# xuqingkuang/FluidFramework

Hardware: AMD Instinct MI355X
Metric: sequenced merge-tree ops applied/sec (node) at 100K docs; % HBM roofline (higher is better)
Workload: dtype int32; 1 GPU; C3: 100000 docs/GPU x 32 clients x 1024 sequenced ops/doc (BASELINE.json configs[2]), full merge-tree apply incl. zamboni; docs_total=100000, docs_per_gpu=100000, docs_rank0=100000, ops_per_doc=1024, ops_per_launch=32, parallelism=hash-routed docs x1 (splitmix64(docId) mod 1; no collective in apply), comm=LocalComm

## Files before the change

fluidframework_amd/build.py:

```python
import os
import subprocess
import sys

HERE = os.path.dirname(os.path.abspath(__file__))
CSRC = os.path.join(HERE, 'csrc')
LIB = os.path.join(HERE, 'libmtgpu.so')
SOURCES = ['mt_apply.hip', 'mt_apply_reg.hip', 'mt_service.hip', 'mt_refs.hip', 'mt_intervals.hip', 'mt_text.hip', 'mt_markers.hip', 'mt_deli.hip', 'mt_engine.cpp',
           'mt_queries.cpp', 'mt_readout.cpp', 'mt_comm.cpp']
HEADERS = ['mt_state.h', 'mt_wave.h', 'mt_checksum.h', 'mt_synth.h', 'mt_seqwin.h', 'mt_view.h', 'mt_marker.h', 'mt_launch.h',
           'mt_engine_impl.h', 'mt_scratch.h', '../../include/mtgpu.h']
HIPCC = os.environ.get('HIPCC', '/opt/rocm/bin/hipcc')
ARCH = os.environ.get('PYTORCH_ROCM_ARCH', 'gfx950')


def needs_build():
    if not os.path.exists(LIB):
        return True
    t = os.path.getmtime(LIB)
    return any(os.path.getmtime(os.path.join(CSRC, f)) > t for f in SOURCES + HEADERS
               if os.path.exists(os.path.join(CSRC, f)))


def build(force=False, verbose=False, prof=False):
    lib = LIB.replace('libmtgpu.so', 'libmtgpu_prof.so') if prof else LIB
    if not prof and not force and not needs_build():
        return LIB
    from concurrent.futures import ThreadPoolExecutor
    objdir = os.path.join(HERE, 'build')
    os.makedirs(objdir, exist_ok=True)
    srcs = [f for f in SOURCES if os.path.exists(os.path.join(CSRC, f))]
    flags = [f'--offload-arch={ARCH}', '-O3', '-std=c++17', '-fPIC', '-Wall', '-Wno-unused-function',
             '-Wno-unused-result', '-Wno-unused-value'] + os.environ.get('MTGPU_EXTRA_FLAGS', '').split()

    stamp = ' '.join(flags + (['-DMT_PROF'] if prof else []))
    hdr_t = max(os.path.getmtime(os.path.join(CSRC, h)) for h in HEADERS if os.path.exists(os.path.join(CSRC, h)))

    def fresh(f, obj):
        try:
            t = os.path.getmtime(obj)
            with open(obj + '.flags') as fh:
                same = fh.read() == stamp
        except OSError:
            return False
        return same and t > os.path.getmtime(os.path.join(CSRC, f)) and t > hdr_t

    def cc(f):
        obj = os.path.join(objdir, f + ('.prof.o' if prof else '.o'))
        if not force and fresh(f, obj):
            return obj
        cmd = [HIPCC] + flags + (['-DMT_PROF'] if prof else []) + ['-c', os.path.join(CSRC, f), '-o', obj]
        if verbose:
            print(' '.join(cmd))
        subprocess.check_call(cmd)
        with open(obj + '.flags', 'w') as fh:
            fh.write(stamp)
        return obj

    with ThreadPoolExecutor(max_workers=len(srcs)) as ex:
        objs = list(ex.map(cc, srcs))
    subprocess.check_call([HIPCC, f'--offload-arch={ARCH}', '-shared', '-o', lib + '.tmp'] + objs +
                          ['-L/opt/rocm/lib', '-lrccl', '-Wl,-rpath,/opt/rocm/lib'])
    os.replace(lib + '.tmp', lib)
    return lib
# ... 28 lines not shown
```

fluidframework_amd/csrc/mt_apply_reg.hip:

```cpp
#include <hip/hip_runtime.h>
#include <stdint.h>

#include "../../include/mtgpu.h"
#include "mt_seqwin.h"
#include "mt_launch.h"
#include "mt_state.h"
#include "mt_wave.h"

namespace mtr {

constexpr int kMaxNodes = 8;
constexpr int kTextGranularity = 256;
constexpr int kNarrowClients = 32;
constexpr int kC64Clients = 63;
constexpr uint32_t kLenBits = 17;
constexpr uint32_t kLenMask = (1u << kLenBits) - 1;
constexpr uint32_t kNoId = 0x7FFFu;
constexpr uint32_t kEmptyLi = kNoId << kLenBits;
constexpr uint32_t F_RM = (uint32_t)MT_SF_REMOVED << 16;
constexpr uint32_t F_PDEF = (uint32_t)MT_SF_PDEF << 16;
constexpr uint32_t F_NL = (uint32_t)MT_SF_NL << 16;
constexpr uint32_t F_HASNL = (uint32_t)MT_SF_HASNL << 16;
constexpr uint32_t F_MARKER = (uint32_t)MT_SF_MARKER << 16;
constexpr uint32_t F_NLQ = 1u << 21;
constexpr uint32_t kEmptyCf = 0xFFu;
constexpr uint32_t kOrgShift = 22;
constexpr uint16_t kDead = 0xFFFFu;

#define MT_GLOB __attribute__((address_space(1)))
#define MT_KARG __attribute__((address_space(4)))
template <class T>
MT_DEV MT_GLOB T* gp(T* p) { return (MT_GLOB T*)p; }
typedef const MT_KARG mt_gstate KGState;
typedef uint32_t EvWords __attribute__((ext_vector_type(4)));
MT_DEV void put_event(MT_GLOB mt_event* p, int32_t seq, int op, unsigned flags, int leaf, int pos, uint32_t len,
                      uint32_t pmask = 0, uint32_t pv01 = 0, uint32_t pv23 = 0, uint32_t pv45 = 0, uint32_t pv67 = 0) {
    static_assert(sizeof(mt_event) == 96 && offsetof(mt_event, pvals) == 24, "mt_event");
    MT_GLOB EvWords* q = reinterpret_cast<MT_GLOB EvWords*>(p);
    const EvWords z = {0u, 0u, 0u, 0u};
    q[0] = EvWords{(uint32_t)seq, ((uint32_t)op & 0xFFu) | ((flags & 0xFFu) << 8), (uint32_t)leaf, (uint32_t)pos};
    q[1] = EvWords{len, pmask, pv01, pv23};
    q[2] = EvWords{pv45, pv67, 0u, 0u};
    q[3] = z;
    q[4] = z;
    q[5] = z;
}

MT_DEV int uni(int v) { return __builtin_amdgcn_readfirstlane(v); }
MT_DEV uint32_t uniu(uint32_t v) { return (uint32_t)__builtin_amdgcn_readfirstlane((int)v); }
MT_DEV int shr1(int v, int fill) { return __builtin_amdgcn_update_dpp(fill, v, 0x138, 0xf, 0xf, false); }
MT_DEV int shl1(int v, int fill) { return __builtin_amdgcn_update_dpp(fill, v, 0x130, 0xf, 0xf, false); }
MT_DEV int wave_total(int v) { return wave_last(wave_incl_scan(v)); }

enum { P_LOAD, P_SCAN, P_BOUND, P_INSERT, P_RANGE, P_ZAMBONI, P_SCOUR, P_STORE, P_OPS, P_ZPOP, P_REPACK,
       P_B_GET, P_B_BLK, P_B_TXT, P_B_INS, P_N_SCOUR, P_N_UNLINK, P_N_APPEND, P_N_SPLIT,
       P_COMPACT, P_N_COMPACT, P_N_APPBYTES, P_B_SRCH, P_B_LEAF, P_OP, P_NSLOT };
[[maybe_unused]] constexpr int kProfStride = 32;
#ifdef MT_PROF
__device__ unsigned long long mt_prof_acc[16 * kProfStride];
MT_DEV uint64_t prof_now() {
    unsigned long long t;
    __builtin_amdgcn_sched_barrier(0);
    asm volatile("s_memtime %0\n\ts_waitcnt lgkmcnt(0)" : "=s"(t)::"memory");
    __builtin_amdgcn_sched_barrier(0);
    return t;
}
#ifndef MT_PROF_ONLY
#define MT_PROF_ONLY -1
#endif
#define PROF_ON(s) (MT_PROF_ONLY < 0 || MT_PROF_ONLY == (s))
#define PROF_BEGIN(v, s) const uint64_t v = PROF_ON(s) ? prof_now() : 0
#define PROF_BEGIN2(v, s1, s2) const uint64_t v = (PROF_ON(s1) || PROF_ON(s2)) ? prof_now() : 0
#define PROF_END(arr, slot, v) \
    do {                       \
        if (PROF_ON(slot)) arr[slot] += prof_now() - (v); \
    } while (0)
#define PROF_CNT(slot, v) prof[slot] += (v)
#else
#define PROF_BEGIN(v, s)
#define PROF_BEGIN2(v, s1, s2)
#define PROF_END(arr, slot, v)
#define PROF_CNT(slot, v)
#endif

template <int K>
struct RLds {
    static constexpr int CAP = 64 * K;
    static constexpr int LB = CAP / 2 > 128 ? CAP / 2 : 128;
    static constexpr int IB = CAP / 8 + 8 > 40 ? CAP / 8 + 8 : 40;
    static constexpr int H = CAP / 2 + 64 > 192 ? CAP / 2 + 64 : 192;
    uint64_t props[CAP];
    union {
        int32_t scr[CAP + 1];
        uint32_t tln[CAP + 1];
    };
    int32_t hseq[H];
    uint16_t toff[CAP];
    uint16_t hslot[H];
    uint8_t ibcnt[MT_MAXLEV - 1][IB];
    uint8_t lbsc[LB + 1];
    int32_t nb[MT_MAXLEV];
    uint32_t zr[4 * kMaxNodes];
    uint64_t dum[64];
};

struct Elem {
    uint32_t sw;
    uint32_t rsq;
    uint32_t li, cf, ov, oh;
    int32_t cum;
};
struct Cut {
    uint32_t lli, lcf, rli;
    int32_t pos;
};

template <int K, bool W = false, bool EV = false>
struct RWave {
    using L = RLds<K>;
    static constexpr int CAP = L::CAP;
    static constexpr uint32_t kAll = (1u << K) - 1u;
    typedef int32_t VI __attribute__((ext_vector_type(K)));
    typedef uint32_t VU __attribute__((ext_vector_type(K)));
    typedef uint32_t U4 __attribute__((ext_vector_type(4)));
    typedef uint32_t U2 __attribute__((ext_vector_type(2)));
    L& s;
    const int lane;
    uint8_t* const abase;
    const uint32_t textcap;

    static constexpr bool PK = K > MT_SW_EXACT_K;
    VU sw;
    VU rsq;
    VU li, cf, ov;
    VU oh;
    VI cum;
    int ns, nlive, nb0, nlev, heap_n, cur_seq, min_seq, err, err_seq, next_id;
    int32_t base_seq;
    uint32_t text_top, text_half;
    bool dirty;
    uint32_t pb;
    uint32_t bsm, lvm, sc0, sc1;
    MT_GLOB mt_event* evp = nullptr;
    uint32_t evcap = 0;
    int evn = 0;
    int32_t evseq = 0;
#ifdef MT_PROF
    uint64_t prof[P_NSLOT] = {};
#endif

    MT_DEV RWave(L& lds, uint8_t* a, uint32_t tc)
        : s(lds), lane(lane_id()), abase(a), textcap(tc), dirty(false) {}
    MT_DEV uint8_t* arena() const { return abase + (size_t)text_half * textcap; }

    MT_DEV int idx(int j) const { return lane * K + j; }

    MT_DEV void fail(int code, int32_t sq) {
        if (err == 0) {
            err = code;
            err_seq = sq;
        }
    }
    MT_DEV static uint32_t len_of(uint32_t l) { return l & kLenMask; }
    MT_DEV static uint32_t id_of(uint32_t l) { return l >> kLenBits; }
    MT_DEV uint32_t lim_of(int32_t R) const { return PK ? mt_sw_lim(R, base_seq) : (uint32_t)R; }
    MT_DEV uint32_t key_of(int32_t S) const { return PK ? mt_sw_off(S, base_seq) : (uint32_t)S; }
    MT_DEV static bool key_le(uint32_t a, uint32_t lim) { return PK ? a <= lim : (int32_t)a <= (int32_t)lim; }
    MT_DEV bool seq_le(int j, uint32_t lim) const { return PK ? mt_sw_seq_le(sw[j], lim) != 0 : (int32_t)sw[j] <= (int32_t)lim; }
    MT_DEV bool rseq_le(int j, uint32_t lim) const { return PK ? mt_sw_rseq_le(sw[j], lim) != 0 : (int32_t)rsq[j] <= (int32_t)lim; }
    MT_DEV bool rseq_eq(int j, uint32_t key) const { return PK ? mt_sw_rseq_eq(sw[j], key) != 0 : rsq[j] == key; }

    MT_DEV uint32_t bs_bits() const { return bsm; }
    MT_DEV uint32_t live_bits() const { return lvm; }
    MT_DEV uint32_t kbit(int k) const {
        const int r = k - lane * K;
        return (r >= 0 && r < K) ? (1u << r) : 0u;
    }
    MT_DEV int sc_of(int a) const {
        const int r = uni(a % K);
        return __builtin_amdgcn_readlane((int)(((sc0 >> r) & 1u) | (((sc1 >> r) & 1u) << 1)), a / K);
    }
    MT_DEV void set_sc(int a, int v) {
        const uint32_t b = kbit(a);
        sc0 = (v & 1) ? (sc0 | b) : (sc0 & ~b);
        sc1 = (v & 2) ? (sc1 | b) : (sc1 & ~b);
    }
    MT_DEV void set_bs(int a, bool on) {
        const uint32_t b = kbit(a);
        bsm = on ? (bsm | b) : (bsm & ~b);
    }
    MT_DEV static uint32_t shift_mask(uint32_t m, uint32_t lo, bool at, bool above, int r, bool bit) {
        const uint32_t c = (uint32_t)shr1((int)((m >> (K - 1)) & 1u), 0);
        return (m & lo) | (((m & ~lo) << 1) & kAll) | ((at && bit) ? (1u << r) : 0u) | (above ? c : 0u);
    }
    MT_DEV void mask_shift(int p, bool bs, int scv, bool live) {
        const uint32_t lo = below(p);
        const int r = p - lane * K;
        const bool at = r >= 0 && r < K, above = r < 0;
        bsm = shift_mask(bsm, lo, at, above, r, bs);
        lvm = shift_mask(lvm, lo, at, above, r, live);
        sc0 = shift_mask(sc0, lo, at, above, r, (scv & 1) != 0);
        sc1 = shift_mask(sc1, lo, at, above, r, (scv & 2) != 0);
    }
    MT_DEV uint32_t below(int k) const {
        const int r = k - lane * K;
        return r <= 0 ? 0u : (r >= K ? kAll : ((1u << r) - 1u));
    }
    MT_DEV int nth_slot(uint32_t m, int r) const {
// ... 317 lines not shown

    MT_DEV bool insert_at(int k, int a, int en, const Elem& e, int32_t sq, const Cut& cut, bool dup) {
        if (ns + 1 > CAP) return fail(MT_DERR_CAPACITY, sq), false;
        const bool front = !dup && k == a;
        PROF_BEGIN(ti0, P_B_INS);
        const int scv = front ? sc_of(a) : 0;
        shift_in<true>(k, e, front, scv, true, dup);
        if (dup) patch_cut(k, cut);
        if (front) {
            set_bs(k + 1, false);
            set_sc(k + 1, MT_SC_UNDEF);
        }
        PROF_END(prof, P_B_INS, ti0);
        nlive += 1;
        PROF_BEGIN(ti1, P_B_LEAF);
        const bool over = live_in(a, en + 1) >= kMaxNodes;
        PROF_END(prof, P_B_LEAF, ti1);
        if (!over) return true;
        PROF_BEGIN(ti2, P_COMPACT);
        PROF_CNT(P_N_COMPACT, 1);
        const bool r = split_leaf(a, en + 1, sq);
        PROF_END(prof, P_COMPACT, ti2);
        return r;
    }
    MT_DEV int alloc_id(int32_t sq) {
        if (next_id >= CAP) {
            fail(MT_DERR_CAPACITY, sq);
            return -1;
        }
        return next_id++;
    }

    MT_DEV void arena_sync() {
        if (dirty) {
            __threadfence_block();
            dirty = false;
        }
    }
    MT_DEV void arena_copy(uint32_t dst, uint32_t src, uint32_t cnt) {
        arena_sync();
        for (uint32_t base = 0; base < cnt; base += 64) {
            const uint32_t i = base + lane;
            if (i < cnt) arena()[dst + i] = arena()[src + i];
        }
        dirty = true;
    }
    MT_DEV void compact_text(int nid) {
        PROF_BEGIN(tc, P_COMPACT);
        PROF_CNT(P_N_COMPACT, 1);
        arena_sync();
        const uint8_t* src0 = arena();
        uint8_t* dst = abase + (size_t)(text_half ^ 1u) * textcap;
        uint32_t carry = 0;
        for (int base = 0; base < nid; base += 64) {
            const int i = base + lane;
            const uint32_t l = i < nid ? s.tln[i] : 0u;
            const uint32_t incl = (uint32_t)wave_incl_scan((int)l);
            const uint32_t at = carry + incl - l;
            if (l) {
                const uint8_t* src = src0 + s.toff[i];
#pragma clang loop unroll(disable) vectorize(disable)
                for (uint32_t q = 0; q < l; q++) dst[at + q] = src[q];
                s.toff[i] = (uint16_t)at;
            }
            carry += (uint32_t)wave_last((int)incl);
        }
        dirty = true;
        wave_sync();
        text_half ^= 1u;
        text_top = carry;
        PROF_END(prof, P_COMPACT, tc);
    }
    MT_DEV bool arena_reserve(uint32_t need, int32_t sq, int nid) {
        if (text_top + need <= textcap) return true;
        compact_text(nid);
        if (text_top + need <= textcap) return true;
        fail(MT_DERR_TEXT_ARENA, sq);
        return false;
    }

    MT_DEV bool split_prep(int pos, int32_t sq, Cut& c, int& k1, int& ba, int& be) {
        PROF_BEGIN(ts0, P_B_SRCH);
        int cs = cs0();
        int hitj = -1;
#pragma unroll
        for (int j = 0; j < K; j++) {
            if (cs < pos && pos < cum[j]) hitj = j;
            cs = cum[j];
        }
        const uint64_t m = wave_ballot(hitj >= 0);
        PROF_END(prof, P_B_SRCH, ts0);
        if (!m) return false;
        PROF_CNT(P_N_SPLIT, 1);
        PROF_BEGIN(tb0, P_B_GET);
        const int lk = first_lane(m);
        const int jk = uni(__builtin_amdgcn_readlane(hitj, lk));
        const int k = lk * K + jk;
        const uint32_t eli = (uint32_t)__builtin_amdgcn_readlane((int)li[jk], lk);
        const uint32_t ecf = (uint32_t)__builtin_amdgcn_readlane((int)cf[jk], lk);
        const int32_t ecum = __builtin_amdgcn_readlane(cum[jk], lk);
        PROF_END(prof, P_B_GET, tb0);
        const uint32_t len = len_of(eli);
        const int off = pos - (ecum - (int)len);
        const int t = alloc_id(sq);
        if (t < 0) return false;
        PROF_BEGIN(tb1, P_B_BLK);
        ba = block_start(k);
        be = next_start(k);
        PROF_END(prof, P_B_BLK, tb1);
        PROF_BEGIN(tb2, P_B_TXT);
        const uint32_t id = id_of(eli);
        const uint64_t pid = s.props[id];
        const uint32_t to = uniu(s.toff[id]);
        if (lane == 0) {
            s.props[t] = pid;
            s.toff[t] = (uint16_t)(to + (uint32_t)off);
            s.tln[id] = (uint32_t)off;
            s.tln[t] = len - (uint32_t)off;
        }
        c.lli = (uint32_t)off | (id << kLenBits);
        c.lcf = (ecf & F_HASNL) ? ((ecf & ~F_NL) | F_NLQ) : (ecf & ~(F_NL | F_NLQ));
        c.rli = (len - (uint32_t)off) | ((uint32_t)t << kLenBits);
        c.pos = pos;
        wave_sync();
        PROF_END(prof, P_B_TXT, tb2);
        if constexpr (EV) {
            const int lf = live_before(k);
            emit(MT_EV_SPLIT, MT_EVF_FIRST, lf, -1, (uint32_t)off);
            emit(MT_EV_SPLIT, 0u, lf + 1, -1, len - (uint32_t)off);
        }
        k1 = k + 1;
        return true;
    }

    MT_DEV bool heap_push(int32_t key, int id, int32_t sq) {
        if (heap_n + 1 >= L::H) return fail(MT_DERR_CAPACITY, sq), false;
        const int k0 = heap_n + 1;
        const int anc = lane < 31 ? (k0 >> (lane + 1)) : 0;
        const bool has = anc >= 1;
        const int32_t av = has ? s.hseq[anc] : 0;
        const uint16_t as = has ? s.hslot[anc] : (uint16_t)0;
        const int up = first_lane(wave_ballot(!has || av - key <= 0));
        wave_sync();
        if (lane < up) {
            const int child = k0 >> lane;
            s.hseq[child] = av;
            s.hslot[child] = as;
        }
        if (lane == 0) {
            s.hseq[k0 >> up] = key;
            s.hslot[k0 >> up] = (uint16_t)id;
        }
        heap_n = heap_n + 1;
        wave_sync();
        return true;
    }
    MT_DEV int heap_pop() {
        const int cnt = heap_n - 1;
        int k = 1, id = 0;
        int32_t x = 0;
        uint32_t xs = 0;
        const int r = lane + 2;
        const int dep = 31 - __builtin_clz((uint32_t)r);
        for (bool first = true, more = true; more; first = false) {
            const int node = (k << dep) + (r - (1 << dep));
            const bool ok = lane < 62 && node <= cnt;
            const int at = lane < 62 ? (ok ? node : 0) : (lane == 62 ? heap_n : 1);
            const int32_t v = (ok || (first && lane >= 62)) ? s.hseq[at] : 0;
            const uint32_t sl = (ok || (first && lane >= 62)) ? (uint32_t)s.hslot[at] : 0u;
            if (first) {
                id = uni(__builtin_amdgcn_readlane((int)sl, 63));
// ... 31 lines not shown
        wave_sync();
        return id;
    }
    MT_DEV bool add_lru(int a, int id, int32_t sq) {
        if (sc_of(a) != MT_SC_TRUE && sq > cur_seq) {
            set_sc(a, MT_SC_TRUE);
            return heap_push(sq, id, sq);
        }
        return true;
    }

    MT_DEV int slot_of_id(int id) const {
        int hit = -1;
#pragma unroll
        for (int j = 0; j < K; j++)
            if ((int)id_of(li[j]) == id && ((lvm >> j) & 1u)) hit = idx(j);
        const uint64_t m = wave_ballot(hit >= 0);
        if (!m) return -1;
        return __builtin_amdgcn_readlane(hit, first_lane(m));
    }

    MT_DEV void append_run(int p, uint32_t runm, uint32_t vli, uint32_t vcf, uint32_t& hli, uint32_t& hcf) {
        const uint32_t pli = (uint32_t)__builtin_amdgcn_readlane((int)vli, p);
        const uint32_t pid_ = id_of(pli);
        const uint32_t lastq = 31u - (uint32_t)__builtin_clz(runm);
        const bool in_run = lane == p || (lane < 32 && ((runm >> lane) & 1u));
        const uint32_t myl = in_run ? len_of(vli) : 0u;
        const uint32_t incl = (uint32_t)wave_incl_scan((int)myl);
        const uint32_t total = (uint32_t)wave_last((int)incl);
        for (int pass = 0; pass < 2; pass++) {
            const uint32_t myt = in_run ? (uint32_t)s.toff[id_of(vli)] : 0u;
            const uint32_t pt = uniu((uint32_t)__builtin_amdgcn_readlane((int)myt, p));
            const bool adj = __ballot(in_run && myt != pt + (incl - myl)) == 0;
            if (adj) break;
            if (pass == 0) {
                if (!arena_reserve(total, cur_seq, next_id)) return;
                continue;
            }
            const uint32_t top = text_top;
            PROF_CNT(P_N_APPBYTES, total);
            uint64_t pieces = __ballot(in_run);
            while (pieces) {
                const int q = first_lane(pieces);
                pieces &= pieces - 1;
                const uint32_t ql = (uint32_t)__builtin_amdgcn_readlane((int)myl, q);
                const uint32_t qt = (uint32_t)__builtin_amdgcn_readlane((int)myt, q);
                const uint32_t at = top + (uint32_t)__builtin_amdgcn_readlane((int)(incl - myl), q);
                arena_copy(at, qt, ql);
            }
            if (lane == 0) s.toff[pid_] = (uint16_t)top;
            text_top = top + total;
            wave_sync();
        }
        if (lane == 0) s.tln[pid_] = total;
        const uint32_t pcf = (uint32_t)__builtin_amdgcn_readlane((int)vcf, p);
        const uint32_t lcf = (uint32_t)__builtin_amdgcn_readlane((int)vcf, (int)lastq);
        const uint32_t anynl = __ballot(in_run && (vcf & F_HASNL)) ? F_HASNL : 0u;
        hli = total | (pid_ << kLenBits);
        hcf = (pcf & ~F_NL) | (lcf & F_NL) | anynl;
    }

    MT_DEV int scour(int a, int e) {
        const uint32_t lb = live_bits() & below(e) & ~below(a);
        const int c = __popc(lb);
        const int incl = wave_incl_scan(c);
        const int rbase = incl - c;
        const int cnt = wave_last(incl);
        if (cnt > kMaxNodes) return fail(MT_DERR_CAPACITY, cur_seq), cnt;
        uint32_t* const dum = reinterpret_cast<uint32_t*>(s.dum) + lane;
#pragma unroll
        for (int j = 0; j < K; j++) {
            const int q = rbase + __popc(lb & ((1u << j) - 1u));
            uint32_t* const z = ((lb >> j) & 1u) ? &s.zr[q] : dum;
            z[0] = PK ? ((cf[j] & F_RM) ? mt_sw_drseq(sw[j]) : mt_sw_dseq(sw[j])) : ((cf[j] & F_RM) ? rsq[j] : sw[j]);
            z[kMaxNodes] = li[j];
            z[2 * kMaxNodes] = cf[j];
            z[3 * kMaxNodes] = (uint32_t)idx(j);
        }
        wave_sync();
        const bool mine = lane < cnt;
        const int zq = lane & (kMaxNodes - 1);
        const uint32_t r0 = s.zr[zq], r1 = s.zr[kMaxNodes + zq], r2 = s.zr[2 * kMaxNodes + zq],
                       r3 = s.zr[3 * kMaxNodes + zq];
        const uint32_t vsq = mine ? r0 : 0u;
        const uint32_t vli = mine ? r1 : 0u;
        uint32_t vcf = mine ? r2 : 0u;
        const int vslot = mine ? (int)r3 : 0;
        const uint64_t pr = s.props[mine ? id_of(vli) : 0u];
        const uint64_t vpr = mine ? pr : 0ull;
        if (__ballot(mine && (vcf & F_NLQ))) {
            arena_sync();
            if (mine && (vcf & F_NLQ)) {
                const uint8_t c = arena()[(uint32_t)s.toff[id_of(vli)] + len_of(vli) - 1];
                vcf = (vcf & ~(F_NL | F_NLQ)) | (c == '\n' ? F_NL : 0u);
            }
        }
        const uint32_t minSeq = lim_of(min_seq);
        const bool rm = mine && (vcf & F_RM) != 0;
        const uint32_t ql = len_of(vli);
        const bool elig = mine && !rm && key_le(vsq, minSeq) && ql > 0;
        const bool pelig = shr1(elig ? 1 : 0, 0) != 0;
        const uint32_t pcf = (uint32_t)shr1((int)vcf, 0);
        const uint32_t pprl = (uint32_t)shr1((int)(uint32_t)vpr, 0);
        const uint32_t pprh = (uint32_t)shr1((int)(uint32_t)(vpr >> 32), 0);
        const bool a0 = elig && pelig && !((pcf | vcf) & F_MARKER) && !(pcf & F_NL) && ((pcf ^ vcf) & F_PDEF) == 0 && pprl == (uint32_t)vpr &&
                        pprh == (uint32_t)(vpr >> 32);
        const uint32_t a0m = (uint32_t)__ballot(a0);
// ... 16 lines not shown
        const int kept = cnt - __popc(unlink);
        const uint32_t heads = ~appm & ((1u << (lane & 31)) - 1u);
        const int vtgt = (lane < 32 && ((appm >> lane) & 1u)) ? 31 - __builtin_clz(heads) : -1;
        if constexpr (EV) {
            const bool app = vtgt >= 0;
            const bool tomb = mine && ((unlink >> lane) & 1u) && !app;
            const int kb = lane - __popc(unlink & (lane < 32 ? ((1u << lane) - 1u) : 0xFFFFFFFFu));
            const int nrec = tomb ? 1 : (app ? 2 : 0);
            const int rinc = wave_incl_scan(nrec);
            const int rtot = wave_last(rinc);
            if (rtot) {
                const int st = live_before(a);
                const int ainc = wave_incl_scan(app ? (int)ql : 0);
                const int hp = app ? vtgt : lane;
                const int kbp = __shfl(kb, hp, 64), aincp = __shfl(ainc, hp, 64);
                const uint32_t lenp = (uint32_t)__shfl((int)ql, hp, 64);
                const int o = evn + rinc - nrec;
                if (tomb && o < (int)evcap) put_event(evp + o, evseq, MT_EV_UNLINK, MT_EVF_FIRST, st + kb, -1, ql);
                if (app) {
                    if (o < (int)evcap)
                        put_event(evp + o, evseq, MT_EV_APPEND, MT_EVF_FIRST, st + kbp, -1, lenp + (uint32_t)(ainc - aincp));
                    if (o + 1 < (int)evcap) put_event(evp + o + 1, evseq, MT_EV_APPEND, 0u, st + kb, -1, ql);
                }
                evn = evn + rtot;
            }
        }
        PROF_CNT(P_N_UNLINK, __popc(unlink));
        uint64_t runs = __ballot(vtgt >= 0);
        if (runs) {
            uint32_t nli = vli, ncf = vcf, heads = 0;
            while (runs) {
                const int p = __builtin_amdgcn_readlane(vtgt, first_lane(runs));
                const uint64_t runm = __ballot(vtgt == p);
                runs &= ~runm;
                PROF_CNT(P_N_APPEND, __popcll(runm));
                uint32_t hli = 0, hcf = 0;
                append_run(p, (uint32_t)runm, vli, vcf, hli, hcf);
                if (err) return cnt;
                nli = lane == p ? hli : nli;
                ncf = lane == p ? hcf : ncf;
                heads |= 1u << p;
            }
#pragma unroll
            for (int j = 0; j < K; j++) {
                const int q = rbase + __popc(lb & ((1u << j) - 1u));
                const bool hit = ((lb >> j) & 1u) && q < 32 && ((heads >> q) & 1u);
                const uint32_t xl = (uint32_t)__builtin_amdgcn_ds_bpermute(q << 2, (int)nli);
                const uint32_t xc = (uint32_t)__builtin_amdgcn_ds_bpermute(q << 2, (int)ncf);
                li[j] = hit ? xl : li[j];
                cf[j] = hit ? xc : cf[j];
            }
        }
        const bool gone = mine && ((unlink >> lane) & 1u);
        if (gone) s.tln[id_of(vli)] = 0u;
        uint64_t gm = __ballot(gone);
        uint32_t kill = 0;
        while (gm) {
            const int sl = __builtin_amdgcn_readlane(vslot, first_lane(gm));
            gm &= gm - 1;
            if (sl / K == lane) kill |= 1u << (sl % K);
        }
        lvm &= ~kill;
        nlive -= __popc(unlink);
        return kept;
    }

    MT_DEV void repack(int Lv, int P, int first_child, int m, int total) {
        for (;;) {
            const int half = kMaxNodes / 2;
            int cc = min(kMaxNodes - 1, total / half);
            if (cc < 1) cc = 1;
            const int base = total / cc, extra = total % cc;
            uint8_t* a = lvl(Lv);
            const int nb = nbl(Lv);
            wave_sync();
            if (cc < m) {
                lshift_left(a, first_child + m, nb, m - cc);
            } else if (cc > m) {
                for (int q = 0; q < cc - m; q++) lshift_right(a, first_child + m, nb + q);
            }
            if (lane < cc) a[first_child + lane] = (uint8_t)(base + (lane < extra ? 1 : 0));
            wave_sync();
            if (lane == 0) {
                s.nb[Lv] = nb + cc - m;
                lvl(Lv + 1)[P] = (uint8_t)cc;
            }
            wave_sync();
            if (!(cc < kMaxNodes / 2 && (Lv + 1) < nlev - 1)) return;
            int fc = 0;
            const int PP = parent_of(Lv + 1, P, &fc);
            Lv = Lv + 1;
            P = PP;
            first_child = fc;
            m = uni(lvl(Lv + 1)[P]);
            total = 0;
            const uint8_t* c = lvl(Lv);
            for (int j = first_child; j < first_child + m; j++) total += uni(c[j]);
        }
    }
    MT_DEV void repack_leaf(int P, int fc, int m, int total, int A, int E) {
        const int half = kMaxNodes / 2;
        int cc = min(kMaxNodes - 1, total / half);
        if (cc < 1) cc = 1;
        const int base = total / cc, extra = total % cc;
        const uint32_t rng = below(E) & ~below(A);
        bsm &= ~rng;
        sc0 &= ~rng;
// ... 83 lines not shown
        } else {
        int first = 0x7fffffff;
#pragma unroll
        for (int j = K - 1; j >= 0; j--) {
            const int i = idx(j);
            first = ((i < ns) & (cum[j] >= pos)) ? i : first;
        }
        first = first_hit(first);
        if (first == 0x7fffffff) return fail(MT_DERR_INSERT_FAILED, S), -1;
        const int a = block_start(first), e = next_start(first);
        ba = a;
        be = e;
        int best = 0x7fffffff;
        {
            const uint32_t Rw = lim_of(R);
            const int cs = cs0();
#pragma unroll
            for (int j = K - 1; j >= 0; j--) {
                const int i = idx(j);
                const int ce = cum[j];
                const int csj = j ? cum[j - 1] : cs;
                const bool rm_before = ((cf[j] & F_RM) != 0) & rseq_le(j, Rw);
                const bool h = (((lvm >> j) & 1u) != 0) & (i >= a) & (i < e) &
                               ((ce > pos) | ((ce == pos) & (csj == pos) & !rm_before));
                best = h ? i : best;
            }
        }
        best = first_hit(best);
        k = best != 0x7fffffff ? best : e;
        }
        const int t = alloc_id(S);
        if (t < 0) return -1;
        if (!arena_reserve((uint32_t)tlen, S, t)) return -1;
        const uint32_t top = text_top;
        bool hasnl = false;
        uint8_t* const ar = arena();
        for (int base = 0; base < tlen; base += 64) {
            const int i = base + lane;
            const uint8_t c = i < tlen ? (uint8_t)(base == 0 ? pb : pay[i]) : 0;
            if (i < tlen) ar[top + i] = c;
            hasnl = hasnl || __ballot(i < tlen && c == '\n') != 0;
        }
        dirty = true;
        uint32_t fl = (op.flags & MT_F_MARKER) ? F_MARKER
                                               : ((pbyte(pay, tlen - 1) == '\n' ? F_NL : 0u) | (hasnl ? F_HASNL : 0u));
        uint64_t p = 0;
        if (op.flags & MT_F_PROPS) {
            fl |= F_PDEF;
            p = apply_pairs(0, pay, tlen, np);
        }
        if (lane == 0) {
            s.props[t] = p;
            s.toff[t] = (uint16_t)top;
            s.tln[t] = (uint32_t)tlen;
        }
        text_top = top + (uint32_t)tlen;
        wave_sync();
        en.sw = PK ? mt_sw_pack(mt_sw_off(S, base_seq), 0u) : (uint32_t)S;
        en.rsq = 0;
        en.li = (uint32_t)tlen | ((uint32_t)t << kLenBits);
        en.cf = (uint32_t)C | fl;
        en.ov = 0;
        en.oh = 0;
        en.cum = pos + tlen;
        return t;
    }

    MT_DEV void range_action(const mt_op_rec op, const uint8_t* pay, int tlen, int np) {
        const int32_t S = op.seq;
        const int C = op.client, start = op.pos1, end = op.pos2;
        const bool is_remove = op.type == MT_OP_REMOVE;
        const bool rewrite = op.flags & MT_F_REWRITE;
        const uint32_t cbit = 1u << ((C - 1) & 31);
        const bool hic = W && C > kNarrowClients;
        uint64_t pclr = 0, pset = 0;
        if (!is_remove) {
            for (int q = 0; q < np; q++) {
                const int k = (int)pbyte(pay, tlen + 2 * q);
                const uint64_t m = 0xFFull << (8 * k);
                pclr |= m;
                pset = (pset & ~m) | ((uint64_t)pbyte(pay, tlen + 2 * q + 1) << (8 * k));
            }
        }
        const uint32_t dS = key_of(S);
        uint32_t tm = 0;
        {
            int cs = cs0();
#pragma unroll
            for (int j = 0; j < K; j++) {
                const int ce = cum[j];
                tm |= (ce > cs && cs < end && ce > start) ? (1u << j) : 0u;
                cs = ce;
            }
        }
        if (EV && !is_remove) emit_range(false, S, C, tm, pclr, pset, rewrite);
        if (is_remove) {
#pragma unroll
            for (int j = 0; j < K; j++) {
                const bool touched = (tm >> j) & 1u;
                const uint32_t f = cf[j];
                const bool was_rm = (f & F_RM) != 0;
                const bool mark = touched && !was_rm;
                const bool overlap = touched && was_rm;
                ov[j] = (overlap && !hic) ? (ov[j] | cbit) : ov[j];
                if constexpr (W) oh[j] = (overlap && hic) ? (oh[j] | cbit) : oh[j];
                if constexpr (PK) sw[j] = mark ? mt_sw_with_drseq(sw[j], dS) : sw[j];
                else rsq[j] = mark ? dS : rsq[j];
// ... 249 lines not shown
        if constexpr (EV) {
            evp = gp(g.ev) + (size_t)d * g.evcap;
            evcap = g.evcap;
            evn = uni((int)gp(g.evn)[d]);
            evseq = cur_seq;
        }
        const size_t so = (size_t)d * g.segcap;
        const size_t lo = (size_t)d * g.lbcap;
        const size_t ho = (size_t)d * g.hcap;
        const int i0 = lane * K;
        const bool mine = i0 < n;
        const int ir = mine ? i0 : 0;
        VU vsq, vrs, vln, vto;
        uint32_t pw[2 * K], ow[2 * K], bcw[BW], brw[BW], bfw[BW];
        vsq = ld_u32(reinterpret_cast<const MT_GLOB uint32_t*>(gp(g.seq) + so + ir));
        vrs = ld_u32(reinterpret_cast<const MT_GLOB uint32_t*>(gp(g.rseq) + so + ir));
        vln = ld_u32(gp(g.len) + so + ir);
        vto = ld_u32(gp(g.toff) + so + ir);
        ld64_raw(gp(g.props) + so + ir, pw);
        ld64_raw(gp(g.ovl) + so + ir, ow);
        ld8_raw(gp(g.client) + so + ir, bcw);
        ld8_raw(gp(g.rclient) + so + ir, brw);
        ld8_raw(gp(g.flags) + so + ir, bfw);
        constexpr int LBC = (L::LB + 63) / 64;
        uint32_t lbc_[LBC], lbs_[LBC];
#pragma unroll
        for (int c = 0; c < LBC; c++) {
            const size_t b = lo + (c * 64 < nb0 ? c * 64 + lane : 0);
            lbc_[c] = gp(g.lbcnt)[b];
            lbs_[c] = gp(g.lbscour)[b];
        }
        constexpr int HC = (L::H + 63) / 64;
        int32_t hq[HC];
        uint32_t hs[HC];
#pragma unroll
        for (int c = 0; c < HC; c++) {
            const size_t i = ho + 1 + (c * 64 < heap_n ? c * 64 + lane : 0);
            hq[c] = gp(g.hseq)[i];
            hs[c] = gp(g.hslot)[i];
        }
        constexpr int IBL = MT_MAXLEV - 1;
        uint32_t ibw[IBL][2];
#pragma unroll
        for (int Lv = 1; Lv <= IBL; Lv++) {
            const size_t io = ((size_t)d * (MT_MAXLEV - 1) + (Lv < nlev ? Lv - 1 : 0)) * g.ibcap;
#pragma unroll
            for (int c = 0; c < 2; c++) ibw[Lv - 1][c] = gp(g.ibcnt)[io + c * 64 + lane];
        }
        __builtin_amdgcn_sched_barrier(0);
#pragma unroll
        for (int j = 0; j < K; j++) {
            s.props[i0 + j] = (uint64_t)pw[2 * j] | ((uint64_t)pw[2 * j + 1] << 32);
            s.toff[i0 + j] = (uint16_t)vto[j];
            s.scr[i0 + j] = 0;
        }
#pragma unroll
        for (int c = 0; c < HC; c++) {
            const int i = 1 + c * 64 + lane;
            if (c * 64 < heap_n && i <= heap_n) {
                s.hseq[i] = hq[c];
                s.hslot[i] = (uint16_t)hs[c];
            }
        }
#pragma unroll
        for (int Lv = 1; Lv <= IBL; Lv++) {
            if (Lv < nlev) {
                const int nbl_ = uni(sc.nb[Lv]);
#pragma unroll
                for (int c = 0; c < 2; c++)
                    if (c * 64 + lane < nbl_) s.ibcnt[Lv - 1][c * 64 + lane] = (uint8_t)ibw[Lv - 1][c];
                if (nbl_ > 128) {
                    const size_t io = ((size_t)d * (MT_MAXLEV - 1) + (Lv - 1)) * g.ibcap;
#pragma clang loop unroll(disable) vectorize(disable)
                    for (int i = 128 + lane; i < nbl_; i += 64) s.ibcnt[Lv - 1][i] = gp(g.ibcnt)[io + i];
                }
            }
        }
        if (lane < MT_MAXLEV) s.nb[lane] = sc.nb[lane];
        wave_sync();
        int nempty = 0;
        {
            int carry = 0;
#pragma unroll
            for (int cc = 0; cc < LBC; cc++) {
                if (cc * 64 < nb0) {
                    const int b = cc * 64 + lane;
                    const int c = b < nb0 ? (int)lbc_[cc] : 0;
                    const int scv = (int)lbs_[cc];
                    const int incl = wave_incl_scan(c) + carry;
                    if (b < nb0 && c > 0) s.scr[incl - c] = 1 | (scv << 1);
                    nempty += __popcll(wave_ballot(b < nb0 && c == 0));
                    carry = wave_last(incl);
                }
            }
        }
        wave_sync();
        bool wide_sq = false;
        bsm = lvm = sc0 = sc1 = 0u;
#pragma unroll
        for (int j = 0; j < K; j++) {
            const bool in = i0 + j < n;
            const bool rmj = (byte_at(bfw, j) & MT_SF_REMOVED) != 0;
            const int mk = s.scr[i0 + j];
            const uint32_t ds = mt_sw_off((int32_t)vsq[j], base_seq);
            const uint32_t dr = rmj ? mt_sw_off((int32_t)vrs[j], base_seq) : 0u;
            if constexpr (PK) {
                sw[j] = in ? mt_sw_pack(ds, dr) : mt_sw_pack(MT_SW_PAD, 0u);
                wide_sq |= in & ((ds > MT_SW_MAX) | (dr > MT_SW_MAX));
            } else {
                sw[j] = in ? vsq[j] : 0x7fffffffu;
                rsq[j] = in ? vrs[j] : 0u;
            }
            li[j] = in ? (vln[j] | ((uint32_t)(i0 + j) << kLenBits)) : kEmptyLi;
            ov[j] = in ? ((ow[2 * j] >> 1) | (ow[2 * j + 1] << 31)) : 0u;
            if constexpr (W) oh[j] = in ? (ow[2 * j + 1] >> 1) : 0u;
            cf[j] = in ? (byte_at(bcw, j) | (byte_at(brw, j) << 8) | ((byte_at(bfw, j) & 0x1Fu) << 16) |
                          (PK ? (uint32_t)(i0 + j) << kOrgShift : 0u))
                       : kEmptyCf;
            cum[j] = 0;
            const uint32_t bit = in ? (1u << j) : 0u;
            lvm |= bit;
            bsm |= (mk & 1) ? bit : 0u;
            sc0 |= (mk & 2) ? bit : 0u;
            sc1 |= (mk & 4) ? bit : 0u;
        }
        if (__ballot(wide_sq)) {
            if (lane == 0) {
                gp(g.sc)[d].err = MT_DERR_LIMITS;
                gp(g.sc)[d].err_seq = cur_seq;
            }
            return false;
        }
        wave_sync();
#pragma unroll
        for (int j = 0; j < K; j++) s.tln[i0 + j] = vln[j];
        if (nempty) {
            if (ns + nempty > CAP) {
                fail(MT_DERR_CAPACITY, cur_seq);
            } else {
                int carry = 0, placed = 0;
                for (int base = 0; base < nb0; base += 64) {
                    const int b = base + lane;
                    const int c = b < nb0 ? (int)gp(g.lbcnt)[lo + b] : 0;
                    const int scv = b < nb0 ? (int)gp(g.lbscour)[lo + b] : 0;
                    const int incl = wave_incl_scan(c) + carry;
                    uint64_t em = wave_ballot(b < nb0 && c == 0);
                    while (em) {
                        const int fl = first_lane(em);
                        em &= em - 1;
                        Elem ph;
                        ph.sw = PK ? mt_sw_pack(MT_SW_PAD, 0u) : 0x7fffffffu;
                        ph.rsq = 0;
                        ph.li = kEmptyLi;
                        ph.cf = kEmptyCf;
                        ph.ov = 0;
                        ph.oh = 0;
                        ph.cum = 0;
                        shift_in<false>(__builtin_amdgcn_readlane(incl - c, fl) + placed, ph, true,
                                        __builtin_amdgcn_readlane(scv, fl), false);
                        placed++;
                    }
                    carry = wave_last(incl);
                }
            }
        }
        return true;
    }

    template <class T, class F>
    MT_DEV void store_field(const T& v, uint32_t lb, int pbase, int nn, F&& put) {
        int32_t* const dum = reinterpret_cast<int32_t*>(s.dum) + lane;
#pragma unroll
        for (int j = 0; j < K; j++)
            *(((lb >> j) & 1u) ? &s.scr[pbase + __popc(lb & ((1u << j) - 1u))] : dum) = (int32_t)v[j];
        wave_sync();
#pragma clang loop unroll(disable) vectorize(disable)
        for (int base = 0; base < nn; base += 256) {
            uint32_t v[4];
#pragma unroll
            for (int q = 0; q < 4; q++) v[q] = (uint32_t)s.scr[min(base + 64 * q + lane, CAP)];
#pragma unroll
            for (int q = 0; q < 4; q++)
                if (base + 64 * q + lane < nn) put(base + 64 * q + lane, v[q]);
        }
        wave_sync();
    }

    MT_DEV void store(KGState& g, uint32_t d) {
        const size_t so = (size_t)d * g.segcap;
        const uint32_t lb = live_bits();
        const int c = __popc(lb);
        const int incl = wave_incl_scan(c);
        const int pbase = incl - c;
        const int nn = wave_last(incl);
        {
            uint32_t q = 0;
#pragma unroll
            for (int j = 0; j < K; j++) q |= ((cf[j] & F_NLQ) && ((lb >> j) & 1u)) ? (1u << j) : 0u;
            if (__ballot(q != 0)) {
                arena_sync();
                uint32_t at[K];
#pragma unroll
                for (int j = 0; j < K; j++) {
                    const bool on = (q >> j) & 1u;
                    const uint32_t to = s.toff[on ? id_of(li[j]) : 0u];
                    at[j] = on ? to + len_of(li[j]) - 1 : 0u;
                }
                uint32_t ch[K];
#pragma unroll
                for (int j = 0; j < K; j++) ch[j] = arena()[at[j]];
#pragma unroll
                for (int j = 0; j < K; j++)
                    if ((q >> j) & 1u) cf[j] = (cf[j] & ~(F_NL | F_NLQ)) | (ch[j] == '\n' ? F_NL : 0u);
            }
        }
        VU xs, xr;
        if constexpr (PK) {
            uint32_t as_[K], ar_[K];
#pragma unroll
            for (int j = 0; j < K; j++) {
                const bool on = (lb >> j) & 1u;
                const uint32_t org = cf[j] >> kOrgShift;
                const bool ns_ = on && mt_sw_dseq(sw[j]) == 0u;
                const bool nr_ = on && (cf[j] & F_RM) && mt_sw_drseq(sw[j]) == 0u;
                as_[j] = (uint32_t)gp(g.seq)[so + (ns_ ? org : 0u)];
                ar_[j] = (uint32_t)gp(g.rseq)[so + (nr_ ? org : 0u)];
            }
#pragma unroll
            for (int j = 0; j < K; j++) {
                xs[j] = (uint32_t)mt_sw_exact(mt_sw_dseq(sw[j]), base_seq, (int32_t)as_[j]);
                xr[j] = (cf[j] & F_RM) ? (uint32_t)mt_sw_exact(mt_sw_drseq(sw[j]), base_seq, (int32_t)ar_[j]) : 0u;
            }
        } else {
            xs = sw;
            xr = rsq;
        }
        store_field(xs, lb, pbase, nn, [&](int i, uint32_t v) { gp(g.seq)[so + i] = (int32_t)v; });
        store_field(xr, lb, pbase, nn, [&](int i, uint32_t v) { gp(g.rseq)[so + i] = (int32_t)v; });
        store_field(ov, lb, pbase, nn, [&](int i, uint32_t v) { gp(g.ovl)[so + i] = (uint64_t)v << 1; });
        if constexpr (W)
            store_field(oh, lb, pbase, nn, [&](int i, uint32_t v) { gp(g.ovl)[so + i] |= (uint64_t)v << 33; });
        store_field(cf, lb, pbase, nn, [&](int i, uint32_t v) {
            gp(g.client)[so + i] = (uint8_t)(v & 0xFFu);
            gp(g.rclient)[so + i] = (uint8_t)((v >> 8) & 0xFFu);
            gp(g.flags)[so + i] = (uint8_t)((v >> 16) & 0x1Fu);
        });
        store_field(li, lb, pbase, nn, [&](int i, uint32_t v) {
            const uint32_t id = id_of(v);
            gp(g.len)[so + i] = len_of(v);
            gp(g.toff)[so + i] = s.toff[id];
            gp(g.props)[so + i] = s.props[id];
        });
        const uint32_t bm = bs_bits();
        const int bc = __popc(bm);
        const int bbase = wave_incl_scan(bc) - bc;
#pragma unroll
        for (int j = 0; j < K; j++) {
            if ((bm >> j) & 1u) {
                const int b = bbase + __popc(bm & ((1u << j) - 1u));
                s.scr[b] = pbase + __popc(lb & ((1u << j) - 1u));
                s.lbsc[b] = (uint8_t)(((sc0 >> j) & 1u) | (((sc1 >> j) & 1u) << 1));
            }
        }
        if (lane == 0) s.scr[nb0] = nn;
        wave_sync();
        const size_t lo = (size_t)d * g.lbcap;
        int nempty = 0;
#pragma clang loop unroll(disable) vectorize(disable)
        for (int b = lane; b < nb0; b += 64) {
            const int cnt = s.scr[b + 1] - s.scr[b];
            gp(g.lbcnt)[lo + b] = (uint8_t)cnt;
            gp(g.lbscour)[lo + b] = s.lbsc[b];
            nempty += cnt == 0 ? 1 : 0;
        }
        nempty = wave_total(nempty);
#pragma clang loop unroll(disable) vectorize(disable)
        for (int i = lane; i < next_id; i += 64) s.toff[i] = kDead;
        wave_sync();
#pragma unroll
        for (int j = 0; j < K; j++)
            if ((lb >> j) & 1u) s.toff[id_of(li[j])] = (uint16_t)(pbase + __popc(lb & ((1u << j) - 1u)));
        wave_sync();
        for (int Lv = 1; Lv < nlev; Lv++) {
            const size_t io = ((size_t)d * (MT_MAXLEV - 1) + (Lv - 1)) * g.ibcap;
            const int nbl_ = min(nbl(Lv), (int)g.ibcap);
#pragma clang loop unroll(disable) vectorize(disable)
            for (int i = lane; i < nbl_; i += 64) gp(g.ibcnt)[io + i] = s.ibcnt[Lv - 1][i];
        }
        if (heap_n >= (int)g.hcap) fail(MT_DERR_CAPACITY, cur_seq);
        const size_t ho = (size_t)d * g.hcap;
        const int hn = min(heap_n, (int)g.hcap - 1);
#pragma clang loop unroll(disable) vectorize(disable)
        for (int i = 1 + lane; i <= hn; i += 64) {
            gp(g.hseq)[ho + i] = s.hseq[i];
            const uint16_t id = s.hslot[i];
            gp(g.hslot)[ho + i] = id == kDead ? kDead : s.toff[id];
        }
        if (lane == 0) {
            MT_GLOB mt_doc_scalars& sc = gp(g.sc)[d];
            sc.nseg = nn;
            sc.nlev = nlev;
            sc.heap_n = heap_n;
            sc.cur_seq = cur_seq;
            sc.min_seq = min_seq;
            sc.err = err;
            sc.err_seq = err_seq;
            sc.text_top = text_top;
            sc.text_half = text_half;
            sc.n_empty = (uint32_t)nempty;
            sc.nb[0] = nb0;
        }
        if (lane >= 1 && lane < MT_MAXLEV) gp(g.sc)[d].nb[lane] = s.nb[lane];
        if constexpr (EV)
            if (lane == 0) gp(g.evn)[d] = (uint32_t)evn;
    }
};

MT_DEV uint32_t load_op_block(const mt_op_rec* ops, uint32_t base, uint32_t end, int lane) {
    const uint32_t r = min(base + (uint32_t)(lane >> 3), end - 1u);
    return reinterpret_cast<const uint32_t*>(ops + r)[lane & 7];
}
MT_DEV uint32_t load_payload(const uint8_t* payload, uint32_t poff, uint32_t plen, int lane) {
    return payload[plen ? poff + min((uint32_t)lane, plen - 1u) : 0u];
}
MT_DEV mt_op_rec op_from_block(uint32_t blk, uint32_t j) {
    const int l = (int)(j * 8);
    mt_op_rec r;
    r.seq = __builtin_amdgcn_readlane((int)blk, l + 0);
    r.ref_seq = __builtin_amdgcn_readlane((int)blk, l + 1);
    r.msn = __builtin_amdgcn_readlane((int)blk, l + 2);
    const uint32_t w3 = (uint32_t)__builtin_amdgcn_readlane((int)blk, l + 3);
    r.client = (uint16_t)(w3 & 0xFFFFu);
    r.type = (uint8_t)((w3 >> 16) & 0xFFu);
    r.flags = (uint8_t)(w3 >> 24);
    r.pos1 = __builtin_amdgcn_readlane((int)blk, l + 4);
    r.pos2 = __builtin_amdgcn_readlane((int)blk, l + 5);
    r.payload_off = (uint32_t)__builtin_amdgcn_readlane((int)blk, l + 6);
    r.payload_len = (uint32_t)__builtin_amdgcn_readlane((int)blk, l + 7);
    return r;
}

MT_DEV KGState& kernarg_gstate() {
    KGState* p = (KGState*)__builtin_amdgcn_kernarg_segment_ptr();
    asm volatile("" : "+s"(p));
    return *p;
}

constexpr int wpe_default(int K) {
    return K <= 3 ? 7 : K <= 5 ? 5 : K <= 8 ? 4 : K <= 12 ? 3 : 2;
}
#ifndef MT_WPE_OV
#define MT_WPE_OV {0}
#endif
constexpr int wpe_ov[17] = MT_WPE_OV;
constexpr int wpe(int K) { return K < 17 && wpe_ov[K] > 0 ? wpe_ov[K] : wpe_default(K); }
template <int K, bool W, bool EV>
MT_DEV void reg_apply(uint8_t* text, uint32_t textcap, const mt_op_rec* __restrict__ ops,
                      const uint8_t* __restrict__ payload, const uint32_t* __restrict__ row_ptr,
                      const uint32_t* __restrict__ doc_ids, uint32_t n_docs, uint32_t op_lo, uint32_t op_cnt) {
    extern __shared__ __attribute__((aligned(16))) unsigned char smem[];
    const uint32_t w = blockIdx.x;
    if (w >= n_docs) return;
    const uint32_t d = doc_ids ? doc_ids[w] : w;
    RLds<K>& lds = *reinterpret_cast<RLds<K>*>(smem);
    RWave<K, W, EV> wv(lds, text + (size_t)d * 2 * textcap, textcap);
    const uint32_t r0 = row_ptr[d], r1 = row_ptr[d + 1];
    const uint32_t a = min(r1, r0 + op_lo);
    const uint32_t b = op_cnt ? min(r1, a + op_cnt) : r1;
    if (a >= b) return;
    PROF_BEGIN(tl, P_LOAD);
    const bool loaded = wv.load(kernarg_gstate(), d);
    PROF_END(wv.prof, P_LOAD, tl);
    if (!loaded) return;
    uint32_t blk0 = load_op_block(ops, a, b, wv.lane);
    uint32_t blk1 = load_op_block(ops, a + 8, b, wv.lane);
    uint32_t pb = load_payload(payload, (uint32_t)__builtin_amdgcn_readlane((int)blk0, 6),
                               (uint32_t)__builtin_amdgcn_readlane((int)blk0, 7), wv.lane);
    uint32_t pbn = 0;
    if (a + 1 < b)
        pbn = load_payload(payload, (uint32_t)__builtin_amdgcn_readlane((int)blk0, 14),
                           (uint32_t)__builtin_amdgcn_readlane((int)blk0, 15), wv.lane);
    for (uint32_t i = a; i < b; i++) {
        if (wv.err) break;
        const mt_op_rec op = op_from_block(blk0, (i - a) & 7u);
        wv.pb = pb;
        PROF_BEGIN(top, P_OP);
        wv.apply(op, payload);
        PROF_END(wv.prof, P_OP, top);
#ifdef MT_PROF
        wv.prof[P_OPS]++;
#endif
        pb = pbn;
        const uint32_t jn = (i + 1 - a) & 7u;
        if (jn == 0) {
            blk0 = blk1;
            blk1 = load_op_block(ops, i + 9, b, wv.lane);
        }
        if (i + 2 < b) {
            const uint32_t j2 = (i + 2 - a) & 7u;
            uint32_t poff, plen;
            if (j2 == 0) {
                poff = (uint32_t)__builtin_amdgcn_readlane((int)blk1, 6);
// ... 118 lines not shown
```

Before: 338.1 million ops/s.

## Shrink per-wave LDS by aliasing scratch into props and 16-bit text lengths

Repacks the register-path LDS struct so large-K variants alias the scan scratch inside the props array, store text lengths as 16-bit with a single tracked 'big' overflow slot, and overlay lbsc onto zr/dum. Props are written out to global memory before the scratch reuse clobbers them. The aim is to cut LDS per wave so more waves fit per CU (the static_asserts target 16/14/13/12 waves for K=9..12), and the waves-per-EU default for K=9 is raised from 3 to 4. This adds bookkeeping for lengths of 65536 or more and depends on the aliasing being ordered correctly.

```diff
diff --git a/fluidframework_amd/build.py b/fluidframework_amd/build.py
--- a/fluidframework_amd/build.py
+++ b/fluidframework_amd/build.py
@@ -8,7 +8,7 @@
 SOURCES = ['mt_apply.hip', 'mt_apply_reg.hip', 'mt_service.hip', 'mt_refs.hip', 'mt_intervals.hip', 'mt_text.hip', 'mt_markers.hip', 'mt_deli.hip', 'mt_engine.cpp',
            'mt_queries.cpp', 'mt_readout.cpp', 'mt_comm.cpp']
 HEADERS = ['mt_state.h', 'mt_wave.h', 'mt_checksum.h', 'mt_synth.h', 'mt_seqwin.h', 'mt_view.h', 'mt_marker.h', 'mt_launch.h',
-           'mt_engine_impl.h', 'mt_scratch.h', '../../include/mtgpu.h']
+           'mt_engine_impl.h', 'mt_scratch.h', 'mt_reg_lds.h', '../../include/mtgpu.h']
 HIPCC = os.environ.get('HIPCC', '/opt/rocm/bin/hipcc')
 ARCH = os.environ.get('PYTORCH_ROCM_ARCH', 'gfx950')
 
diff --git a/fluidframework_amd/csrc/mt_apply_reg.hip b/fluidframework_amd/csrc/mt_apply_reg.hip
--- a/fluidframework_amd/csrc/mt_apply_reg.hip
+++ b/fluidframework_amd/csrc/mt_apply_reg.hip
@@ -4,12 +4,12 @@
 #include "../../include/mtgpu.h"
 #include "mt_seqwin.h"
 #include "mt_launch.h"
+#include "mt_reg_lds.h"
 #include "mt_state.h"
 #include "mt_wave.h"
 
 namespace mtr {
 
-constexpr int kMaxNodes = 8;
 constexpr int kTextGranularity = 256;
 constexpr int kNarrowClients = 32;
 constexpr int kC64Clients = 63;
@@ -83,27 +83,6 @@
 #define PROF_CNT(slot, v)
 #endif
 
-template <int K>
-struct RLds {
-    static constexpr int CAP = 64 * K;
-    static constexpr int LB = CAP / 2 > 128 ? CAP / 2 : 128;
-    static constexpr int IB = CAP / 8 + 8 > 40 ? CAP / 8 + 8 : 40;
-    static constexpr int H = CAP / 2 + 64 > 192 ? CAP / 2 + 64 : 192;
-    uint64_t props[CAP];
-    union {
-        int32_t scr[CAP + 1];
-        uint32_t tln[CAP + 1];
-    };
-    int32_t hseq[H];
-    uint16_t toff[CAP];
-    uint16_t hslot[H];
-    uint8_t ibcnt[MT_MAXLEV - 1][IB];
-    uint8_t lbsc[LB + 1];
-    int32_t nb[MT_MAXLEV];
-    uint32_t zr[4 * kMaxNodes];
-    uint64_t dum[64];
-};
-
 struct Elem {
     uint32_t sw;
     uint32_t rsq;
@@ -154,6 +133,15 @@
     MT_DEV uint8_t* arena() const { return abase + (size_t)text_half * textcap; }
 
     MT_DEV int idx(int j) const { return lane * K + j; }
+    using TL = typename L::tln_t;
+    MT_DEV TL* tln() const {
+        if constexpr (L::SCR_OWN) return s.tln32;
+        else return s.tln16;
+    }
+    MT_DEV int32_t* scr() const {
+        if constexpr (L::SCR_OWN) return s.scr_own;
+        else return s.scr_props;
+    }
 
     MT_DEV void fail(int code, int32_t sq) {
         if (err == 0) {
@@ -577,9 +565,10 @@
         const uint8_t* src0 = arena();
         uint8_t* dst = abase + (size_t)(text_half ^ 1u) * textcap;
         uint32_t carry = 0;
+        const int big = L::SCR_OWN ? -1 : uni(s.big);
         for (int base = 0; base < nid; base += 64) {
             const int i = base + lane;
-            const uint32_t l = i < nid ? s.tln[i] : 0u;
+            const uint32_t l = i < nid ? (i == big ? 65536u : (uint32_t)tln()[i]) : 0u;
             const uint32_t incl = (uint32_t)wave_incl_scan((int)l);
             const uint32_t at = carry + incl - l;
             if (l) {
@@ -640,8 +629,9 @@
         if (lane == 0) {
             s.props[t] = pid;
             s.toff[t] = (uint16_t)(to + (uint32_t)off);
-            s.tln[id] = (uint32_t)off;
-            s.tln[t] = len - (uint32_t)off;
+            tln()[id] = (TL)off;
+            tln()[t] = (TL)(len - (uint32_t)off);
+            if (!L::SCR_OWN && (len >> 16)) s.big = -1;
         }
         c.lli = (uint32_t)off | (id << kLenBits);
         c.lcf = (ecf & F_HASNL) ? ((ecf & ~F_NL) | F_NLQ) : (ecf & ~(F_NL | F_NLQ));
@@ -779,7 +769,10 @@
             text_top = top + total;
             wave_sync();
         }
-        if (lane == 0) s.tln[pid_] = total;
+        if (lane == 0) {
+            tln()[pid_] = (TL)total;
+            if (!L::SCR_OWN && (total >> 16)) s.big = (int32_t)pid_;
+        }
         const uint32_t pcf = (uint32_t)__builtin_amdgcn_readlane((int)vcf, p);
         const uint32_t lcf = (uint32_t)__builtin_amdgcn_readlane((int)vcf, (int)lastq);
         const uint32_t anynl = __ballot(in_run && (vcf & F_HASNL)) ? F_HASNL : 0u;
@@ -902,7 +895,10 @@
             }
         }
         const bool gone = mine && ((unlink >> lane) & 1u);
-        if (gone) s.tln[id_of(vli)] = 0u;
+        if (gone) {
+            tln()[id_of(vli)] = 0;
+            if (!L::SCR_OWN && (ql >> 16)) s.big = -1;
+        }
         uint64_t gm = __ballot(gone);
         uint32_t kill = 0;
         while (gm) {
@@ -1092,7 +1088,8 @@
         if (lane == 0) {
             s.props[t] = p;
             s.toff[t] = (uint16_t)top;
-            s.tln[t] = (uint32_t)tlen;
+            tln()[t] = (TL)tlen;
+            if (!L::SCR_OWN && (tlen >> 16)) s.big = t;
         }
         text_top = top + (uint32_t)tlen;
         wave_sync();
@@ -1448,8 +1445,9 @@
         for (int j = 0; j < K; j++) {
             s.props[i0 + j] = (uint64_t)pw[2 * j] | ((uint64_t)pw[2 * j + 1] << 32);
             s.toff[i0 + j] = (uint16_t)vto[j];
-            s.scr[i0 + j] = 0;
-        }
+            tln()[i0 + j] = 0;
+        }
+        if (lane == 0) s.big = -1;
 #pragma unroll
         for (int c = 0; c < HC; c++) {
             const int i = 1 + c * 64 + lane;
@@ -1484,7 +1482,7 @@
                     const int c = b < nb0 ? (int)lbc_[cc] : 0;
                     const int scv = (int)lbs_[cc];
                     const int incl = wave_incl_scan(c) + carry;
-                    if (b < nb0 && c > 0) s.scr[incl - c] = 1 | (scv << 1);
+                    if (b < nb0 && c > 0) tln()[incl - c] = (TL)(1 | (scv << 1));
                     nempty += __popcll(wave_ballot(b < nb0 && c == 0));
                     carry = wave_last(incl);
                 }
@@ -1497,7 +1495,7 @@
         for (int j = 0; j < K; j++) {
             const bool in = i0 + j < n;
             const bool rmj = (byte_at(bfw, j) & MT_SF_REMOVED) != 0;
-            const int mk = s.scr[i0 + j];
+            const int mk = tln()[i0 + j];
             const uint32_t ds = mt_sw_off((int32_t)vsq[j], base_seq);
             const uint32_t dr = rmj ? mt_sw_off((int32_t)vrs[j], base_seq) : 0u;
             if constexpr (PK) {
@@ -1529,7 +1527,10 @@
         }
         wave_sync();
 #pragma unroll
-        for (int j = 0; j < K; j++) s.tln[i0 + j] = vln[j];
+        for (int j = 0; j < K; j++) {
+            tln()[i0 + j] = (TL)vln[j];
+            if (!L::SCR_OWN && i0 + j < n && (vln[j] >> 16)) s.big = i0 + j;
+        }
         if (nempty) {
             if (ns + nempty > CAP) {
                 fail(MT_DERR_CAPACITY, cur_seq);
@@ -1568,13 +1569,13 @@
         int32_t* const dum = reinterpret_cast<int32_t*>(s.dum) + lane;
 #pragma unroll
         for (int j = 0; j < K; j++)
-            *(((lb >> j) & 1u) ? &s.scr[pbase + __popc(lb & ((1u << j) - 1u))] : dum) = (int32_t)v[j];
+            *(((lb >> j) & 1u) ? &scr()[pbase + __popc(lb & ((1u << j) - 1u))] : dum) = (int32_t)v[j];
         wave_sync();
 #pragma clang loop unroll(disable) vectorize(disable)
         for (int base = 0; base < nn; base += 256) {
             uint32_t v[4];
 #pragma unroll
-            for (int q = 0; q < 4; q++) v[q] = (uint32_t)s.scr[min(base + 64 * q + lane, CAP)];
+            for (int q = 0; q < 4; q++) v[q] = (uint32_t)scr()[min(base + 64 * q + lane, CAP)];
 #pragma unroll
             for (int q = 0; q < 4; q++)
                 if (base + 64 * q + lane < nn) put(base + 64 * q + lane, v[q]);
@@ -1609,6 +1610,19 @@
                 for (int j = 0; j < K; j++)
                     if ((q >> j) & 1u) cf[j] = (cf[j] & ~(F_NL | F_NLQ)) | (ch[j] == '\n' ? F_NL : 0u);
             }
+        }
+        if constexpr (!L::SCR_OWN) {
+            VU plo, phi;
+#pragma unroll
+            for (int j = 0; j < K; j++) {
+                const uint64_t p = s.props[((lb >> j) & 1u) ? id_of(li[j]) : 0u];
+                plo[j] = (uint32_t)p;
+                phi[j] = (uint32_t)(p >> 32);
+            }
+            wave_sync();
+            MT_GLOB uint32_t* const pw = reinterpret_cast<MT_GLOB uint32_t*>(gp(g.props) + so);
+            store_field(plo, lb, pbase, nn, [&](int i, uint32_t v) { pw[2 * i] = v; });
+            store_field(phi, lb, pbase, nn, [&](int i, uint32_t v) { pw[2 * i + 1] = v; });
         }
         VU xs, xr;
         if constexpr (PK) {
@@ -1645,7 +1659,7 @@
             const uint32_t id = id_of(v);
             gp(g.len)[so + i] = len_of(v);
             gp(g.toff)[so + i] = s.toff[id];
-            gp(g.props)[so + i] = s.props[id];
+            if constexpr (L::SCR_OWN) gp(g.props)[so + i] = s.props[id];
         });
         const uint32_t bm = bs_bits();
         const int bc = __popc(bm);
@@ -1654,17 +1668,17 @@
         for (int j = 0; j < K; j++) {
             if ((bm >> j) & 1u) {
                 const int b = bbase + __popc(bm & ((1u << j) - 1u));
-                s.scr[b] = pbase + __popc(lb & ((1u << j) - 1u));
+                scr()[b] = pbase + __popc(lb & ((1u << j) - 1u));
                 s.lbsc[b] = (uint8_t)(((sc0 >> j) & 1u) | (((sc1 >> j) & 1u) << 1));
             }
         }
-        if (lane == 0) s.scr[nb0] = nn;
+        if (lane == 0) scr()[nb0] = nn;
         wave_sync();
         const size_t lo = (size_t)d * g.lbcap;
         int nempty = 0;
 #pragma clang loop unroll(disable) vectorize(disable)
         for (int b = lane; b < nb0; b += 64) {
-            const int cnt = s.scr[b + 1] - s.scr[b];
+            const int cnt = scr()[b + 1] - scr()[b];
             gp(g.lbcnt)[lo + b] = (uint8_t)cnt;
             gp(g.lbscour)[lo + b] = s.lbsc[b];
             nempty += cnt == 0 ? 1 : 0;
@@ -1743,7 +1757,7 @@
 }
 
 constexpr int wpe_default(int K) {
-    return K <= 3 ? 7 : K <= 5 ? 5 : K <= 8 ? 4 : K <= 12 ? 3 : 2;
+    return K <= 3 ? 7 : K <= 5 ? 5 : K <= 9 ? 4 : K <= 12 ? 3 : 2;
 }
 #ifndef MT_WPE_OV
 #define MT_WPE_OV {0}
diff --git a/fluidframework_amd/csrc/mt_reg_lds.h b/fluidframework_amd/csrc/mt_reg_lds.h
--- /dev/null
+++ b/fluidframework_amd/csrc/mt_reg_lds.h
@@ -0,0 +1,49 @@
+#pragma once
+#include <stdint.h>
+
+#include <type_traits>
+
+#include "mt_state.h"
+
+namespace mtr {
+
+constexpr int kMaxNodes = 8;
+
+template <int K>
+struct RLds {
+    static constexpr int CAP = 64 * K;
+    static constexpr int LB = CAP / 2 > 128 ? CAP / 2 : 128;
+    static constexpr int IB = CAP / 8 + 8 > 40 ? CAP / 8 + 8 : 40;
+    static constexpr int H = CAP / 2 + 64 > 192 ? CAP / 2 + 64 : 192;
+    static constexpr bool SCR_OWN = K <= 7;
+    using tln_t = std::conditional_t<SCR_OWN, uint32_t, uint16_t>;
+    union {
+        uint64_t props[CAP];
+        int32_t scr_props[CAP + 1];
+    };
+    union {
+        int32_t scr_own[SCR_OWN ? CAP + 1 : 1];
+        uint32_t tln32[SCR_OWN ? CAP + 1 : 1];
+    };
+    union {
+        struct {
+            uint32_t zr[4 * kMaxNodes];
+            uint64_t dum[64];
+        };
+        uint8_t lbsc[LB + 1];
+    };
+    int32_t hseq[H];
+    int32_t nb[MT_MAXLEV];
+    int32_t big;
+    uint16_t tln16[SCR_OWN ? 1 : CAP];
+    uint16_t toff[CAP];
+    uint16_t hslot[H];
+    uint8_t ibcnt[MT_MAXLEV - 1][IB];
+};
+static_assert(sizeof(RLds<9>) <= 10240, "RLds<9>: 16 waves per CU");
+static_assert(sizeof(RLds<10>) <= 11264, "RLds<10>: 14 waves per CU");
+static_assert(sizeof(RLds<11>) <= 12288 && sizeof(RLds<12>) <= 13312, "RLds<11> / <12>: 13 / 12 waves per CU");
+static_assert(sizeof(RLds<8>::scr_props) <= sizeof(RLds<8>::props) && RLds<2>::LB <= RLds<2>::CAP, "scr inside props");
+static_assert(sizeof(RLds<16>::lbsc) <= sizeof(RLds<16>::zr) + sizeof(RLds<16>::dum), "lbsc inside zr + dum");
+
+}
diff --git a/fluidframework_amd/csrc/mt_reg_lds_sizes.cpp b/fluidframework_amd/csrc/mt_reg_lds_sizes.cpp
--- /dev/null
+++ b/fluidframework_amd/csrc/mt_reg_lds_sizes.cpp
@@ -0,0 +1,11 @@
+#include <cstdio>
+
+#include "mt_reg_lds.h"
+
+template <int K>
+static void row() {
+    std::printf("%d %zu\n", K, sizeof(mtr::RLds<K>));
+    if constexpr (K < 16) row<K + 1>();
+}
+
+int main() { row<2>(); }
```

Measured after the change: 350.7 million ops/s, median of 6. 3.7% higher.
